# faverogian/diffusion-classifier

Measured on AMD Instinct MI355X. Metric: images classified/sec (node), CIFAR-10 10-class x 50-step ELBO scoring, higher is better.
Workload: dtype bf16; 1 GPU; cifar10-unet-10x50; classes=10, trials=50, forwards_per_image=500, input=uniform [-1,1], parallelism=single

## Files before the change

### diffusion-classifier_amd/csrc/igemm.hip

```cpp
#include <stdio.h>
#include <stdlib.h>
#include "conv3_halo_plan.h"

template <typename T, int BM, int BN, int WGM, int WGN>
__global__ __launch_bounds__(256, 2) void igemm_kernel(const IgemmArgs a) {
  constexpr int EPC = Elem<T>::EPC;
  constexpr int BKE = 8 * EPC;
  constexpr int XL = BM / 32;
  constexpr int WL = (BN + 31) / 32;
  constexpr int WTM = BM / WGM, WTN = BN / WGN;
  constexpr int TM = WTM / 16, TN = WTN / 16;
  static_assert(WGM * WGN == 4, "4 waves");
  extern __shared__ __attribute__((aligned(16))) char smem[];
  constexpr int BUF = (BM + BN) * 128;

  const int t = threadIdx.x;
  const int lane = t & 63, wave = t >> 6;
  const int wm = wave / WGN, wn = wave % WGN;
  const int lr = lane & 15, lq = lane >> 4;

  int tile_m, tile_n;
  tile_of_block(a, tile_m, tile_n);

  const int HWo = a.Hout * a.Wout;
  const int pad = (a.taps == 9) ? 1 : 0;
  const int Hs = a.upsample ? (a.Hin >> 1) : a.Hin;
  const int Ws = a.upsample ? (a.Win >> 1) : a.Win;
  const int chunk = t & 7, lrow = t >> 3;

  int ns0[XL], ns1[XL], iy0[XL], ix0[XL];
#pragma unroll
  for (int i = 0; i < XL; ++i) {
    const int m = tile_m * BM + lrow + 32 * i;
    const bool vm = m < a.M;
    const int mm = vm ? m : 0;
    const int n = mm / HWo;
    const int rem = mm - n * HWo;
    const int oy = rem / a.Wout, ox = rem - oy * a.Wout;
    ns0[i] = a.map0 ? a.map0[n] : n;
    ns1[i] = a.src1 ? (a.map1 ? a.map1[n] : n) : 0;
    iy0[i] = vm ? oy * a.stride - pad : -(1 << 20);
    ix0[i] = ox * a.stride - pad;
  }
  const T* wbase = reinterpret_cast<const T*>(a.W) + (size_t)(tile_n * BN + lrow) * a.Ktot + chunk * EPC;

  chunk16 xr[XL], wr[WL];
  const chunk16 zero = {0u, 0u, 0u, 0u};

  auto load_regs = [&](int ks, int tap, int cc) {
    int ky = 0, kx = 0;
    if (a.taps == 9) { ky = tap / 3; kx = tap - ky * 3; }
    const bool s1 = cc >= a.c0chunks;
    const T* src = reinterpret_cast<const T*>(s1 ? a.src1 : a.src0);
    const int ld = s1 ? a.ld1 : a.ld0;
    const int coff = (s1 ? cc - a.c0chunks : cc) * BKE + chunk * EPC;
#pragma unroll
    for (int i = 0; i < XL; ++i) {
      const int iy = iy0[i] + ky, ix = ix0[i] + kx;
      const bool ok = (unsigned)iy < (unsigned)a.Hin && (unsigned)ix < (unsigned)a.Win;
      const int sy = a.upsample ? (iy >> 1) : iy, sx = a.upsample ? (ix >> 1) : ix;
      const size_t pix = ((size_t)(s1 ? ns1[i] : ns0[i]) * Hs + sy) * Ws + sx;
      xr[i] = zero;
      if (ok) xr[i] = *reinterpret_cast<const chunk16*>(src + pix * ld + coff);
    }
#pragma unroll
    for (int i = 0; i < WL; ++i) {
      if (BN >= 32 * (i + 1) || lrow + 32 * i < BN)
        wr[i] = *reinterpret_cast<const chunk16*>(wbase + (size_t)(32 * i) * a.Ktot + (size_t)ks * BKE);
    }
  };
  auto write_lds = [&](int buf) {
    char* Xs = smem + buf * BUF;
    char* Wsm = Xs + BM * 128;
#pragma unroll
    for (int i = 0; i < XL; ++i) *reinterpret_cast<chunk16*>(Xs + lds_off(lrow + 32 * i, chunk)) = xr[i];
#pragma unroll
    for (int i = 0; i < WL; ++i)
      if (BN >= 32 * (i + 1) || lrow + 32 * i < BN)
        *reinterpret_cast<chunk16*>(Wsm + lds_off(lrow + 32 * i, chunk)) = wr[i];
  };

  f32x4 acc[TN][TM];
#pragma unroll
  for (int i = 0; i < TN; ++i)
#pragma unroll
    for (int j = 0; j < TM; ++j) acc[i][j] = f32x4{0.f, 0.f, 0.f, 0.f};

  int tap = 0, cc = 0;
  load_regs(0, 0, 0);
  write_lds(0);
  __syncthreads();
  for (int ks = 0; ks < a.nk; ++ks) {
    const bool more = ks + 1 < a.nk;
    if (more) {
      if (++cc == a.cpt) { cc = 0; ++tap; }
      load_regs(ks + 1, tap, cc);
    }
    const char* Xs = smem + (ks & 1) * BUF;
    const char* Wsm = Xs + BM * 128;
#pragma unroll
    for (int sub = 0; sub < 2; ++sub) {
      const int c = sub * 4 + lq;
      chunk16 xf[TM], wf[TN];
#pragma unroll
      for (int j = 0; j < TM; ++j) xf[j] = *reinterpret_cast<const chunk16*>(Xs + lds_off(wm * WTM + j * 16 + lr, c));
#pragma unroll
      for (int i = 0; i < TN; ++i) wf[i] = *reinterpret_cast<const chunk16*>(Wsm + lds_off(wn * WTN + i * 16 + lr, c));
#pragma unroll
      for (int i = 0; i < TN; ++i)
#pragma unroll
        for (int j = 0; j < TM; ++j) acc[i][j] = Mma<T>::run(wf[i], xf[j], acc[i][j]);
    }
    if (more) write_lds((ks + 1) & 1);
    __syncthreads();
  }

  igemm_epilogue<TM, TN>(a, acc, tile_m * BM + wm * WTM, tile_n * BN + wn * WTN, lr, lq);
}

template <typename T, int BM, int BN, int WGM, int WGN>
static int launch(const IgemmArgs& a, hipStream_t s) {
  constexpr int lds = 2 * (BM + BN) * 128;
  static bool attr_done = false;
  auto kern = igemm_kernel<T, BM, BN, WGM, WGN>;
  if (!attr_done) {
    (void)hipFuncSetAttribute(reinterpret_cast<const void*>(kern), hipFuncAttributeMaxDynamicSharedMemorySize, lds);
    attr_done = true;
  }
  const long long nblk = (long long)a.tiles_m * a.tiles_n;
  if (nblk <= 0 || nblk > 0x7fffffffLL) { dc_set_error("dc_igemm: bad grid %lld", nblk); return DC_ERR_SHAPE; }
  hipLaunchKernelGGL(kern, dim3((unsigned)nblk), dim3(256), lds, s, a);
  return dc_check_launch("dc_igemm");
}

extern "C" int32_t dc_igemm_cout_pad(int32_t cout, int32_t tile_n) {
  const int tn = tile_n == 32 ? 32 : 128;
  return (cout + tn - 1) / tn * tn;
}


static int igemm_validate_and_fill(const dc_igemm_params* p, IgemmArgs& a) {
  DC_REQUIRE(p, DC_ERR_ARG, "dc_igemm: null params");
  DC_REQUIRE(p->dtype == DC_F32 || p->dtype == DC_BF16 || p->dtype == DC_F16, DC_ERR_DTYPE, "dc_igemm: dtype %d", p->dtype);
  DC_REQUIRE(p->taps == 1 || p->taps == 9, DC_ERR_ARG, "dc_igemm: taps must be 1 or 9 (got %d)", p->taps);
  DC_REQUIRE(p->stride == 1 || p->stride == 2, DC_ERR_ARG, "dc_igemm: stride %d", p->stride);
  DC_REQUIRE(p->tile_n == 128 || p->tile_n == 32, DC_ERR_ARG, "dc_igemm: tile_n %d", p->tile_n);
  DC_REQUIRE(p->src0 && p->W && (p->out || p->pn_out), DC_ERR_ARG, "dc_igemm: null src0/W/out");
  const int bke = 128 / dc_dtype_size(p->dtype);
  DC_REQUIRE(p->C0 > 0 && p->C0 % bke == 0, DC_ERR_SHAPE, "dc_igemm: C0=%d not a multiple of %d", p->C0, bke);
  DC_REQUIRE(p->C1 >= 0 && p->C1 % bke == 0 && ((p->C1 > 0) == (p->src1 != nullptr)), DC_ERR_SHAPE,
             "dc_igemm: C1=%d / src1 mismatch or not a multiple of %d", p->C1, bke);
  DC_REQUIRE(p->n_img > 0 && p->Hout > 0 && p->Wout > 0 && p->Hin > 0 && p->Win > 0 && p->Cout > 0, DC_ERR_SHAPE,
             "dc_igemm: non-positive extent");
  if (p->taps == 9) {
    DC_REQUIRE(p->Hout == (p->Hin + 2 - 3) / p->stride + 1 && p->Wout == (p->Win + 2 - 3) / p->stride + 1, DC_ERR_SHAPE,
               "dc_igemm: 3x3 output %dx%d does not match input %dx%d stride %d", p->Hout, p->Wout, p->Hin, p->Win, p->stride);
  } else {
    DC_REQUIRE(p->stride == 1 && !p->upsample && p->Hout == p->Hin && p->Wout == p->Win, DC_ERR_SHAPE,
               "dc_igemm: taps=1 needs stride 1, no upsample, equal in/out extents");
  }
  if (p->upsample) DC_REQUIRE((p->Hin % 2 == 0) && (p->Win % 2 == 0), DC_ERR_SHAPE, "dc_igemm: upsample needs even Hin/Win");
  const long long M = (long long)p->n_img * p->Hout * p->Wout;
  DC_REQUIRE(M < (1LL << 31), DC_ERR_SHAPE, "dc_igemm: M=%lld too large", M);
  DC_REQUIRE(p->act >= 0 && p->act <= 3, DC_ERR_ARG, "dc_igemm: act %d", p->act);
  if (p->act == DC_ACT_GEGLU) DC_REQUIRE(p->Cout % 32 == 0 && p->tile_n == 128, DC_ERR_SHAPE, "dc_igemm: GEGLU needs Cout%%32==0, tile_n 128");
  if (p->act == DC_ACT_GEGLU) DC_REQUIRE(!p->rowvec, DC_ERR_ARG, "dc_igemm: rowvec cannot be combined with DC_ACT_GEGLU");
  if (p->act == DC_ACT_GEGLU) DC_REQUIRE(!p->gate, DC_ERR_ARG, "dc_igemm: gate cannot be combined with DC_ACT_GEGLU");
  DC_REQUIRE(((uintptr_t)p->src0 & 15) == 0 && ((uintptr_t)p->W & 15) == 0 && ((uintptr_t)p->src1 & 15) == 0, DC_ERR_ALIGN,
             "dc_igemm: src/W must be 16-byte aligned");
  const int epc = 16 / dc_dtype_size(p->dtype);
  DC_REQUIRE(p->ld0 % epc == 0 && p->ld1 % epc == 0 && (p->ld0 == 0 || p->ld0 >= p->C0) && (p->ld1 == 0 || p->ld1 >= p->C1),
             DC_ERR_SHAPE, "dc_igemm: ld0=%d ld1=%d", p->ld0, p->ld1);
  const int cout_out = p->act == DC_ACT_GEGLU ? p->Cout / 2 : p->Cout;
  DC_REQUIRE(p->out_ld >= cout_out, DC_ERR_SHAPE, "dc_igemm: out_ld %d < %d", p->out_ld, cout_out);
  if (p->residual) DC_REQUIRE(p->res_ld >= cout_out, DC_ERR_SHAPE, "dc_igemm: res_ld");
  if (p->rowvec) DC_REQUIRE(p->rowvec_ld >= cout_out, DC_ERR_SHAPE, "dc_igemm: rowvec_ld");
  if (p->gate) DC_REQUIRE(p->gate_ld >= cout_out, DC_ERR_SHAPE, "dc_igemm: gate_ld");

  a.src0 = p->src0; a.map0 = p->map0; a.src1 = p->src1; a.map1 = p->map1; a.W = p->W; a.bias = p->bias;
  a.rowvec = p->rowvec; a.rowvec_map = p->rowvec_map; a.gate = p->gate; a.gate_map = p->gate_map;
  a.residual = p->residual; a.res_map = p->res_map; a.out = p->out;
  a.gn_scale = p->gn_scale; a.gn_shift = p->gn_shift; a.gn_silu = p->gn_silu;
  a.src2 = p->src2; a.map2 = p->map2; a.W2 = p->W2; a.C2 = p->C2; a.ld2 = p->ld2 ? p->ld2 : p->C2;
  a.ln_eps = p->ln_eps; a.qstats = p->qstats;
  a.pn_out = p->pn_out; a.pn_gamma = p->pn_gamma; a.pn_beta = p->pn_beta; a.pn_cnt = reinterpret_cast<unsigned*>(p->pn_cnt);
  a.pn_ld = p->pn_ld ? p->pn_ld : p->Cout; a.pn_groups = p->pn_groups; a.pn_silu = p->pn_silu; a.pn_eps = p->pn_eps;
  DC_REQUIRE((p->gn_scale == nullptr) == (p->gn_shift == nullptr), DC_ERR_ARG, "dc_igemm: gn_scale/gn_shift must both be set or null");
  a.C0 = p->C0; a.C1 = p->C1; a.ld0 = p->ld0 ? p->ld0 : p->C0; a.ld1 = p->ld1 ? p->ld1 : p->C1;
  a.rowvec_ld = p->rowvec_ld; a.gate_ld = p->gate_ld; a.res_dtype = p->res_dtype;
  a.res_ld = p->res_ld; a.out_dtype = p->out_dtype; a.out_ld = p->out_ld; a.act = p->act;
  a.taps = p->taps; a.stride = p->stride; a.upsample = p->upsample; a.Hin = p->Hin; a.Win = p->Win;
  a.Hout = p->Hout; a.Wout = p->Wout; a.Cout = p->Cout;
  a.M = (int)M; a.Ktot = p->taps * (p->C0 + p->C1);
  a.c0chunks = p->C0 / bke; a.cpt = (p->C0 + p->C1) / bke; a.nk = p->taps * a.cpt;
  const int bn = p->tile_n;
  a.tiles_m = (a.M + 127) / 128;
  a.tiles_n = dc_igemm_cout_pad(p->Cout, bn) / bn;
  {
    constexpr long long gemm_cap = 16LL << 20;
    const long long wbytes = (long long)dc_igemm_cout_pad(p->Cout, bn) * a.Ktot * dc_dtype_size(p->dtype);
    a.n_fast = (a.tiles_n > 1 && (wbytes <= (2 << 20) || (p->taps == 1 && wbytes <= gemm_cap))) ? 1 : 0;
  }
  return DC_OK;
}

enum IgemmKernel { IG_THIN, IG_WS, IG_HALO, IG_UP4_HALO, IG_UP4_PIPE, IG_XREG, IG_PIPE, IG_REG128, IG_REG32 };

struct IgemmChoice {
  IgemmKernel kernel = IG_REG32;
  int shape = 0;
  bool gn = false, pn = false;
  int status = DC_OK;
  const char* tag = nullptr;
  const char* message = nullptr;
  HaloPlan halo;
};

static IgemmChoice refuse(const char* tag, const char* message) { return IgemmChoice{IG_REG32, 0, false, false, DC_ERR_UNSUPPORTED, tag, message}; }

static IgemmChoice igemm_choose(const dc_igemm_params* p, const IgemmArgs& a) {
  const int dt = p->dtype, bn = p->tile_n, epc = 16 / dc_dtype_size(dt);
  const int cout_out = p->act == DC_ACT_GEGLU ? p->Cout / 2 : p->Cout;
  const bool lane_epi_ok = cout_out % 8 == 0 && p->out_ld % 8 == 0 && ((uintptr_t)p->out & 15) == 0 &&
                           (!p->residual || (p->res_ld % 8 == 0 && ((uintptr_t)p->residual & 15) == 0)) &&
                           (!p->bias || ((uintptr_t)p->bias & 15) == 0) &&
                           (!p->rowvec || (((uintptr_t)p->rowvec & 15) == 0 && p->rowvec_ld % 4 == 0)) &&
                           (!p->gate || (((uintptr_t)p->gate & 15) == 0 && p->gate_ld % 4 == 0 && p->act == DC_ACT_NONE)) &&
                           (!p->residual || p->res_dtype == dt) && (p->out_dtype == dt || p->out_dtype == DC_F32);
  const bool lds_dma = bn == 128 && lane_epi_ok;
  static const bool no_halo = getenv("DCAMD_NO_HALO") != nullptr;
  const bool halo_ok = lds_dma && !no_halo && dc_conv3_halo_applicable(a, dt);
  const bool qs_args_ok = p->out_dtype == dt && p->Cout % 8 == 0 && ((uintptr_t)a.qstats & 15) == 0;
  const bool pn_args_ok = a.pn_gamma && a.pn_beta && a.pn_cnt && p->out_dtype == dt && a.pn_ld % 8 == 0 && a.pn_ld >= p->Cout &&
                          (((uintptr_t)a.pn_out | (uintptr_t)a.qstats) & 15) == 0 && ((uintptr_t)a.pn_cnt & 3) == 0 && a.pn_eps > 0.f;
  const bool use_pn = a.pn_out != nullptr;

  if (p->up4) {
    const bool up4_halo = lds_dma && !no_halo && !a.src1 && dc_conv3_up4_applicable(a, dt) &&
                          (!a.qstats || (qs_args_ok && (a.Hin >> 1) >= 8 && (a.Win >> 1) >= 8));
    const bool up4_pipe = !up4_halo && lds_dma && !a.src1 && !a.qstats && p->taps == 9 && p->stride == 1 &&
                          p->upsample && p->act == DC_ACT_NONE && !p->gate && !p->residual && !a.gn_scale && !a.src2 &&
                          p->Hin >= 4 && p->Win >= 4 && p->Hin % 2 == 0 && p->Win % 2 == 0 && (p->Hin < 16 || p->Win < 16);
    const HaloPlan plan = up4_halo ? dc_conv3_halo_plan(dc_conv3_up4_walked(a), dt, p->n_img, true) : HaloPlan{};
    if (use_pn && !(up4_halo && a.Hin > 16 && a.Win > 16 && dc_conv3_halo_pn_ok(a, plan, true) && a.qstats && pn_args_ok))
      return refuse("producer-groupnorm-unsupported", "dc_igemm: pn_out given but this upsample conv cannot normalise its own output (see dc_igemm_pn_ok)");
    if (!up4_halo && !up4_pipe)
      return refuse("up4-unsupported", "dc_igemm: up4 given but this problem cannot take the four-phase upsample conv (see dc_igemm_up4_ok)");
    if (up4_halo) return IgemmChoice{IG_UP4_HALO, 0, false, use_pn, DC_OK, nullptr, nullptr, plan};
    return IgemmChoice{IG_UP4_PIPE};
  }

  const bool thin_app = dc_conv3_thin_applicable(a, dt);
  const bool thin = thin_app && ((uintptr_t)p->out & 3) == 0;
  static const bool ws_plain = getenv("DCAMD_WS_PLAIN") != nullptr;
  const bool ws_ok = halo_ok && dc_conv3_ws_ok(a, dt) && !thin_app;
  const bool use_ws = ws_ok && (a.gn_scale || ws_plain);
  const HaloPlan plan = halo_ok && !thin && !use_ws ? dc_conv3_halo_plan(a, dt, p->n_img, false) : HaloPlan{};
  const int bke64 = 64 / dc_dtype_size(dt);
  if (a.src2 && !(halo_ok && (!a.gn_scale || ws_ok) && !a.upsample && a.W2 && a.C2 >= 2 * bke64 && a.C2 % bke64 == 0 && a.ld2 % epc == 0 &&
                  (((uintptr_t)a.src2 | (uintptr_t)a.W2) & 15) == 0))
    return refuse("side-source-unsupported", "dc_igemm: src2/W2 given but this problem cannot take the 1x1 side source (see dc_igemm_side_ok)");
  if (a.gn_scale && !thin && !ws_ok)
    return refuse("gn-not-fusable", "dc_igemm: gn_scale/gn_shift given but this problem cannot take the fused GroupNorm prologue (see dc_igemm_gn_fusable)");
  if (a.qstats && !(halo_ok && !thin_app && qs_args_ok && a.Hin >= 8 && a.Win >= 8))
    return refuse("qstats-unsupported", "dc_igemm: qstats given but this problem cannot emit quad statistics (see dc_igemm_qstats_parts)");
  if (use_pn && !(halo_ok && !use_ws && !a.gn_scale && !thin_app && dc_conv3_halo_pn_ok(a, plan, false) &&
                  (a.qstats || (a.Hin == 4 && a.Win == 4)) && pn_args_ok))
    return refuse("producer-groupnorm-unsupported", "dc_igemm: pn_out given but this problem cannot normalise its own output (see dc_igemm_pn_ok)");
  const bool xreg_app = dc_igemm_xreg_applicable(a, dt);
  if (a.ln_eps > 0.f && !(lds_dma && !a.src1 && xreg_app))
    return refuse("row-layernorm-unsupported", "dc_igemm: ln_eps given but this problem cannot take the fused row LayerNorm (see dc_igemm_ln_ok)");

  if (thin) return IgemmChoice{IG_THIN};
  if (use_ws) return IgemmChoice{IG_WS, 0, a.gn_scale != nullptr};
  if (halo_ok) return IgemmChoice{IG_HALO, 0, false, use_pn, DC_OK, nullptr, nullptr, plan};
  if (!lds_dma) return IgemmChoice{bn == 128 ? IG_REG128 : IG_REG32};
  const int shape = dc_igemm_pipe_shape(a);
  if (xreg_app && (p->act == DC_ACT_GEGLU || a.ln_eps > 0.f || shape != 2)) return IgemmChoice{IG_XREG};
  return IgemmChoice{IG_PIPE, shape};
}

static const char* igemm_name(const IgemmChoice& c, int dtype) {
  static const char* const pipe_fmt[3] = {"igemm_pipe<%s,128x128,2st>", "igemm_pipe<%s,256x128,3st>", "igemm_wide8<%s,256x256>"};
  static thread_local char name[64];
  const char* dn = dtype == DC_BF16 ? "bf16" : (dtype == DC_F16 ? "f16" : "f32");
  switch (c.kernel) {
    case IG_THIN: snprintf(name, sizeof(name), "conv3_thin<%s>", dn); break;
    case IG_WS: snprintf(name, sizeof(name), c.gn ? "conv3_ws<%s,gn>" : "conv3_ws<%s>", dn); break;
    case IG_HALO: snprintf(name, sizeof(name), c.pn ? "conv3_halo<%s,%dw,pn>" : "conv3_halo<%s,%dw>", dn, c.halo.key.NW); break;
    case IG_UP4_HALO: snprintf(name, sizeof(name), c.pn ? "conv3_up4<%s,%dw,pn>" : "conv3_up4<%s,%dw>", dn, c.halo.key.NW); break;
    case IG_UP4_PIPE: snprintf(name, sizeof(name), "igemm_pipe_up4<%s,256x128,3st>", dn); break;
    case IG_XREG: snprintf(name, sizeof(name), "igemm_xreg<%s,96xN>", dn); break;
    case IG_PIPE: snprintf(name, sizeof(name), pipe_fmt[c.shape], dn); break;
    case IG_REG128: snprintf(name, sizeof(name), "igemm<%s,128x128>", dn); break;
    case IG_REG32: snprintf(name, sizeof(name), "igemm<%s,128x32>", dn); break;
  }
  return name;
}

static int igemm_launch(const IgemmChoice& c, const IgemmArgs& a, const dc_igemm_params* p, dc_stream stream) {
  hipStream_t s = reinterpret_cast<hipStream_t>(stream);
  switch (c.kernel) {
    case IG_THIN: return dc_conv3_thin_launch(a, p->dtype, p->n_img, s);
    case IG_WS: return dc_conv3_ws_launch(a, p->dtype, p->n_img, s);
    case IG_HALO: return dc_conv3_halo_launch(c.halo, a, p->dtype, false, s);
    case IG_UP4_HALO: return dc_conv3_halo_launch(c.halo, a, p->dtype, true, s);
    case IG_UP4_PIPE: return dc_igemm_launch_pipe_up4(a, p->dtype, s);
    case IG_XREG: return dc_igemm_xreg_launch(a, p->dtype, s);
    case IG_PIPE: return dc_igemm_launch_pipe(a, p->dtype, c.shape, s);
    case IG_REG128: return dc_by_dtype(p->dtype, "dc_igemm: dtype", [&](auto t) { return launch<decltype(t), 128, 128, 2, 2>(a, s); });
    case IG_REG32: return dc_by_dtype(p->dtype, "dc_igemm: dtype", [&](auto t) { return launch<decltype(t), 128, 32, 4, 1>(a, s); });
  }
  return DC_ERR_ARG;
}

extern "C" int dc_igemm(const dc_igemm_params* p, dc_stream stream) {
  IgemmArgs a;
  const int rc = igemm_validate_and_fill(p, a);
  if (rc != DC_OK) return rc;
  const IgemmChoice c = igemm_choose(p, a);
  if (c.status != DC_OK) { dc_set_error("%s", c.message); return c.status; }
  return igemm_launch(c, a, p, stream);
}

extern "C" const char* dc_igemm_variant(const dc_igemm_params* p) {
  IgemmArgs a;
  if (igemm_validate_and_fill(p, a) != DC_OK) return "invalid";
  const IgemmChoice c = igemm_choose(p, a);
  return c.status == DC_OK ? igemm_name(c, p->dtype) : c.tag;
}

extern "C" const char* dc_igemm_instance(const dc_igemm_params* p, int32_t* geom) {
  IgemmArgs a;
  if (igemm_validate_and_fill(p, a) != DC_OK) return "invalid";
  const IgemmChoice c = igemm_choose(p, a);
  if (c.status != DC_OK) return c.tag;
  static thread_local char name[64];
  const char* dn = p->dtype == DC_BF16 ? "bf16" : (p->dtype == DC_F16 ? "f16" : "f32");
  HaloPlan pl;
  switch (c.kernel) {
    case IG_HALO: case IG_UP4_HALO: {
      pl = c.halo;
      const HaloKey& k = pl.key;
      snprintf(name, sizeof(name), "conv3_halo_kernel<%s,%d,%d,%d%s%s>", dn, k.NW, k.NTAP, k.MODE, k.STG ? ",stag" : "", k.PN ? ",pn" : "");
      break;
    }
    case IG_THIN: pl = dc_conv3_thin_plan(a, p->n_img); snprintf(name, sizeof(name), "conv3_thin_kernel<%s,%s>", dn, a.gn_scale ? "gn" : "plain"); break;
    case IG_WS: pl = dc_conv3_ws_plan(a, p->n_img); snprintf(name, sizeof(name), "conv3_ws_kernel<%s,%s>", dn, a.gn_scale ? "gn" : "plain"); break;
    default: return igemm_name(c, p->dtype);
  }
  if (geom) halo_plan_ints(pl, geom);
  return name;
}

static int32_t igemm_accepts(const dc_igemm_params& q) {
  IgemmArgs a;
  return igemm_validate_and_fill(&q, a) == DC_OK && igemm_choose(&q, a).status == DC_OK ? 1 : 0;
}
alignas(16) static float g_probe_dummy[4] = {0.f, 0.f, 0.f, 0.f};

extern "C" int32_t dc_igemm_gn_fusable(const dc_igemm_params* p) {
  if (!p) return 0;
  dc_igemm_params q = *p;
  q.gn_scale = g_probe_dummy; q.gn_shift = g_probe_dummy;
  return igemm_accepts(q);
}

extern "C" int32_t dc_igemm_ln_ok(const dc_igemm_params* p) {
  if (!p) return 0;
  dc_igemm_params q = *p;
  if (!(q.ln_eps > 0.f)) q.ln_eps = 1e-5f;
  return igemm_accepts(q);
}

extern "C" int32_t dc_igemm_qstats_parts(const dc_igemm_params* p) {
  if (!p) return 0;
  dc_igemm_params q = *p;
  if (!q.qstats) q.qstats = g_probe_dummy;
  if (!igemm_accepts(q)) return 0;
  const int hw = p->Hout * p->Wout;
  if (p->up4) { const int lo = hw >> 2; return 4 * (lo >= 128 ? lo / 128 : 1); }
  return hw >= 128 ? hw / 128 : 1;
}

extern "C" int32_t dc_igemm_pn_ok(const dc_igemm_params* p) {
  if (!p || p->pn_groups <= 0) return 0;
  dc_igemm_params q = *p;
  if (!q.pn_out) q.pn_out = g_probe_dummy;
  if (!q.qstats && !(q.Hin == 4 && q.Win == 4)) q.qstats = g_probe_dummy;
  if (!q.pn_gamma) q.pn_gamma = g_probe_dummy;
  if (!q.pn_beta) q.pn_beta = g_probe_dummy;
  if (!q.pn_cnt) q.pn_cnt = reinterpret_cast<uint32_t*>(g_probe_dummy);
  if (!(q.pn_eps > 0.f)) q.pn_eps = 1e-5f;
  return igemm_accepts(q);
}

extern "C" int32_t dc_pn_timeouts(void) { return (int32_t)dc_conv3_halo_pn_timeouts(); }

struct TailChoice { IgemmArgs a; IgemmChoice c; int status = DC_OK; const char* tag = nullptr; const char* message = nullptr; };

static TailChoice tail_choose(const dc_igemm_params* conv, const dc_pn_tail_params* tail, bool probe) {
  TailChoice t;
  auto fail = [&](int st, const char* tag, const char* msg) -> TailChoice& { t.status = st; t.tag = tag; t.message = msg; return t; };
  if (!conv || !tail) return fail(DC_ERR_ARG, "invalid", "dc_conv3_pn_tail: null params");
  if (conv->out || conv->pn_out) return fail(DC_ERR_UNSUPPORTED, "tail-raw-output", "dc_conv3_pn_tail: the conv's own output (out / pn_out) is never stored; leave both null");
  dc_igemm_params q = *conv;
  q.pn_out = g_probe_dummy;
  q.pn_gamma = tail->gamma; q.pn_beta = tail->beta; q.pn_cnt = tail->cnt;
  q.pn_ld = 0; q.pn_groups = tail->groups; q.pn_silu = tail->silu; q.pn_eps = tail->eps;
  if (probe) {
    if (!q.qstats) q.qstats = g_probe_dummy;
    if (!q.pn_gamma) q.pn_gamma = g_probe_dummy;
    if (!q.pn_beta) q.pn_beta = g_probe_dummy;
    if (!q.pn_cnt) q.pn_cnt = reinterpret_cast<uint32_t*>(g_probe_dummy);
    if (!(q.pn_eps > 0.f)) q.pn_eps = 1e-5f;
  } else if (!tail->Wt || !tail->pred || !tail->ring || ((uintptr_t)tail->Wt & 15) || (((uintptr_t)tail->pred | (uintptr_t)tail->ring | (uintptr_t)tail->bias) & 3)) {
    return fail(DC_ERR_ARG, "invalid", "dc_conv3_pn_tail: Wt (16-byte aligned), pred and ring must be given");
  }
  if (q.pn_groups <= 0) return fail(DC_ERR_ARG, "invalid", "dc_conv3_pn_tail: groups");
  if (igemm_validate_and_fill(&q, t.a) != DC_OK) return fail(DC_ERR_ARG, "invalid", nullptr);
  t.c = igemm_choose(&q, t.a);
  if (t.c.status != DC_OK) return fail(t.c.status, t.c.tag, t.c.message);
  if (t.c.kernel != IG_HALO || !t.c.pn || !dc_conv3_halo_tail_ok(t.a, t.c.halo, q.dtype, tail->Co) || tail->pred_ld < tail->Co)
    return fail(DC_ERR_UNSUPPORTED, "tail-unsupported",
                "dc_conv3_pn_tail: needs a 16-bit 3x3 conv with Cout = 128 on the 4-wave producer-GroupNorm form and 1 <= Co <= 3 (see dc_conv3_pn_tail_ok)");
  return t;
}

extern "C" int32_t dc_conv3_pn_tail_ok(const dc_igemm_params* conv, const dc_pn_tail_params* tail) {
  return tail_choose(conv, tail, true).status == DC_OK ? 1 : 0;
}

extern "C" const char* dc_conv3_pn_tail_variant(const dc_igemm_params* conv, const dc_pn_tail_params* tail) {
  const TailChoice t = tail_choose(conv, tail, true);
  if (t.status != DC_OK) return t.tag;
  return conv->dtype == DC_BF16 ? "conv3_halo<bf16,4w,pn,tail>" : "conv3_halo<f16,4w,pn,tail>";
}

extern "C" int64_t dc_conv3_pn_tail_ring_floats(const dc_igemm_params* conv, const dc_pn_tail_params* tail) {
  const TailChoice t = tail_choose(conv, tail, true);
  if (t.status != DC_OK) return 0;
  const HaloGeom& g = t.c.halo.g;
  return (long long)conv->n_img * g.tiles_x * g.tiles_y * PN_TAIL_RING(1 << g.ltw, 1 << g.lth) * tail->Co;
}

extern "C" int dc_conv3_pn_tail(const dc_igemm_params* conv, const dc_pn_tail_params* tail, dc_stream stream) {
  const TailChoice t = tail_choose(conv, tail, false);
  if (t.status != DC_OK) { if (t.message) dc_set_error("%s", t.message); return t.status; }
  hipStream_t s = reinterpret_cast<hipStream_t>(stream);
  const PnTail tl{tail->Wt, tail->bias, tail->pred, tail->ring, tail->Co, tail->pred_ld};
  const int rc = dc_conv3_halo_tail_launch(t.c.halo, t.a, conv->dtype, tl, s);
  if (rc != DC_OK) return rc;
  const HaloGeom& g = t.c.halo.g;
  return dc_pn_tail_combine_launch(tail->pred, tail->ring, conv->n_img, g.ltw, g.lth, g.tiles_x, g.tiles_y, g.H, g.W, tail->Co, tail->pred_ld, s);
}

extern "C" int32_t dc_igemm_up4_ok(const dc_igemm_params* p) {
  if (!p) return 0;
  dc_igemm_params q = *p;
  q.up4 = 1;
  return igemm_accepts(q);
}

extern "C" int32_t dc_igemm_side_ok(const dc_igemm_params* p) {
  if (!p) return 0;
  dc_igemm_params q = *p;
  if (!q.src2) { q.src2 = g_probe_dummy; q.W2 = g_probe_dummy; }
  return igemm_accepts(q);
}
```

### diffusion-classifier_amd/csrc/igemm_common.h

```cpp
#pragma once
#include "common.h"

struct IgemmArgs {
  const void* src0; const int32_t* map0; const void* src1; const int32_t* map1;
  const void* W; const float* bias;
  const float* rowvec; const int32_t* rowvec_map;
  const float* gate; const int32_t* gate_map;
  const void* residual; const int32_t* res_map;
  void* out;
  const float* gn_scale; const float* gn_shift; int gn_silu;
  const void* src2; const int32_t* map2; const void* W2; int C2, ld2;
  float ln_eps;
  float* qstats;
  void* pn_out; const float* pn_gamma; const float* pn_beta; unsigned* pn_cnt; int pn_ld, pn_groups, pn_silu; float pn_eps;
  int C0, C1, ld0, ld1, rowvec_ld, gate_ld, res_dtype, res_ld, out_dtype, out_ld, act;
  int taps, stride, upsample, Hin, Win, Hout, Wout, Cout;
  int M, Ktot, c0chunks, cpt, nk, tiles_m, tiles_n;
  int n_fast;
};

template <typename T> struct Mma;
template <> struct Mma<__bf16> {
  static __device__ __forceinline__ f32x4 run(const chunk16 w, const chunk16 x, f32x4 acc) {
    return __builtin_amdgcn_mfma_f32_16x16x32_bf16(__builtin_bit_cast(bf16x8, w), __builtin_bit_cast(bf16x8, x), acc, 0, 0, 0);
  }
};
template <> struct Mma<_Float16> {
  static __device__ __forceinline__ f32x4 run(const chunk16 w, const chunk16 x, f32x4 acc) {
    return __builtin_amdgcn_mfma_f32_16x16x32_f16(__builtin_bit_cast(f16x8, w), __builtin_bit_cast(f16x8, x), acc, 0, 0, 0);
  }
};
template <> struct Mma<float> {
  static __device__ __forceinline__ f32x4 run(const chunk16 w, const chunk16 x, f32x4 acc) {
    const f32x4 wf = __builtin_bit_cast(f32x4, w), xf = __builtin_bit_cast(f32x4, x);
    acc = __builtin_amdgcn_mfma_f32_16x16x4f32(wf[0], xf[0], acc, 0, 0, 0);
    acc = __builtin_amdgcn_mfma_f32_16x16x4f32(wf[1], xf[1], acc, 0, 0, 0);
    acc = __builtin_amdgcn_mfma_f32_16x16x4f32(wf[2], xf[2], acc, 0, 0, 0);
    acc = __builtin_amdgcn_mfma_f32_16x16x4f32(wf[3], xf[3], acc, 0, 0, 0);
    return acc;
  }
};

__device__ __forceinline__ int lds_off(int row, int chunk) { return row * 128 + ((chunk ^ ((row >> 1) & 7)) << 4); }

__device__ __forceinline__ void tile_of_block(const IgemmArgs& a, int& tile_m, int& tile_n) {
  const int nblk = gridDim.x, bid = blockIdx.x;
  const int q = nblk >> 3, r = nblk & 7, xcd = bid & 7;
  const int lid = (xcd < r ? xcd * (q + 1) : r * (q + 1) + (xcd - r) * q) + (bid >> 3);
  const bool nf = a.n_fast != 0;
  int tn = a.tiles_n, tm = a.tiles_m;
  asm volatile("" : "+s"(tn), "+s"(tm));
  const int d = nf ? tn : tm;
  const int qt = lid / d, rm = lid - qt * d;
  tile_m = nf ? qt : rm;
  tile_n = nf ? rm : qt;
}

template <int TM, int TN>
__device__ __forceinline__ void igemm_epilogue(const IgemmArgs& a, f32x4 (&acc)[TN][TM], int m0, int n0, int lr, int lq) {
  const int HWo = a.Hout * a.Wout;
  const bool geglu = a.act == DC_ACT_GEGLU;
  const int cout_out = geglu ? (a.Cout >> 1) : a.Cout;
#pragma unroll
  for (int j = 0; j < TM; ++j) {
    const int m = m0 + j * 16 + lr;
    if (m >= a.M) continue;
    const int n = m / HWo;
    const float* rv = a.rowvec ? a.rowvec + (size_t)(a.rowvec_map ? a.rowvec_map[n] : n) * a.rowvec_ld : nullptr;
    const float* gt = a.gate ? a.gate + (size_t)(a.gate_map ? a.gate_map[n] : n) * a.gate_ld : nullptr;
    size_t rrow = 0;
    if (a.residual) rrow = (a.res_map ? (size_t)a.res_map[n] * HWo + (m - n * HWo) : (size_t)m) * a.res_ld;
    const size_t orow = (size_t)m * a.out_ld;
#pragma unroll
    for (int i = 0; i < TN; i += 1) {
      const int pc = n0 + i * 16 + lq * 4;
      float v[4];
      int oc;
      if (geglu) {
        if (i & 1) continue;
        oc = ((n0 + i * 16) >> 1) + lq * 4;
        if (oc >= cout_out) continue;
#pragma unroll
        for (int r = 0; r < 4; ++r) {
          float val = acc[i][j][r], g = acc[(i + 1) % TN][j][r];
          if (a.bias) { val += a.bias[pc + r]; g += a.bias[pc + 16 + r]; }
          v[r] = val * gelu_erf_f(g);
        }
      } else {
        oc = pc;
#pragma unroll
        for (int r = 0; r < 4; ++r) {
          float x = acc[i][j][r];
          const int c = oc + r;
          if (c < cout_out) {
            if (a.bias) x += a.bias[c];
            if (rv) x += rv[c];
            if (a.act == DC_ACT_SILU) x = silu_f(x);
            else if (a.act == DC_ACT_GELU_TANH) x = gelu_tanh_f(x);
            if (gt) x *= gt[c];
          }
          v[r] = x;
        }
      }
      if (oc >= cout_out) continue;
      if (a.residual) {
#pragma unroll
        for (int r = 0; r < 4; ++r)
          if (oc + r < cout_out) v[r] += load_as(a.residual, rrow + oc + r, a.res_dtype);
      }
      if (oc + 3 < cout_out && (a.out_ld & 3) == 0) {
        if (a.out_dtype == DC_F32) {
          *reinterpret_cast<float4*>(reinterpret_cast<float*>(a.out) + orow + oc) = make_float4(v[0], v[1], v[2], v[3]);
        } else if (a.out_dtype == DC_BF16) {
          __bf16 h[4] = {(__bf16)v[0], (__bf16)v[1], (__bf16)v[2], (__bf16)v[3]};
          *reinterpret_cast<uint2*>(reinterpret_cast<__bf16*>(a.out) + orow + oc) = *reinterpret_cast<uint2*>(h);
        } else {
          _Float16 h[4] = {(_Float16)v[0], (_Float16)v[1], (_Float16)v[2], (_Float16)v[3]};
          *reinterpret_cast<uint2*>(reinterpret_cast<_Float16*>(a.out) + orow + oc) = *reinterpret_cast<uint2*>(h);
        }
      } else {
#pragma unroll
        for (int r = 0; r < 4; ++r)
          if (oc + r < cout_out) store_as(a.out, orow + oc + r, a.out_dtype, v[r]);
      }
    }
  }
}

int dc_igemm_pipe_shape(const IgemmArgs& a);
int dc_igemm_launch_pipe(const IgemmArgs& a, int dtype, int shape, hipStream_t s);
int dc_igemm_launch_wide8(const IgemmArgs& a, int dtype, hipStream_t s);
__device__ __forceinline__ void tile_of_block_scalar(const IgemmArgs& a, int& tile_m, int& tile_n) {
  tile_of_block(a, tile_m, tile_n);
  tile_m = __builtin_amdgcn_readfirstlane(tile_m);
  tile_n = __builtin_amdgcn_readfirstlane(tile_n);
  asm volatile("" : "+s"(tile_m), "+s"(tile_n));
}

bool dc_conv3_halo_applicable(const IgemmArgs& a, int dtype);
bool dc_conv3_up4_applicable(const IgemmArgs& a, int dtype);
IgemmArgs dc_conv3_up4_walked(const IgemmArgs& a);
int dc_igemm_launch_pipe_up4(const IgemmArgs& a, int dtype, hipStream_t s);
unsigned dc_conv3_halo_pn_timeouts();
bool dc_conv3_ws_ok(const IgemmArgs& a, int dtype);
int dc_conv3_ws_launch(const IgemmArgs& a, int dtype, int n_img, hipStream_t s);
bool dc_igemm_xreg_applicable(const IgemmArgs& a, int dtype);
int dc_igemm_xreg_launch(const IgemmArgs& a, int dtype, hipStream_t s);
bool dc_conv3_thin_applicable(const IgemmArgs& a, int dtype);
int dc_conv3_thin_launch(const IgemmArgs& a, int dtype, int n_img, hipStream_t s);
```

### diffusion-classifier_amd/csrc/igemm_xreg.hip

```cpp
#include <stdlib.h>
#include "igemm_epilogue.h"
DC_CLOCK_DECL(igemm_xreg)
#ifdef DC_XR_STAMPS
static __device__ unsigned long long* g_xr_stamps;
extern "C" void dc_debug_set_xr_stamps(unsigned long long* p) { (void)hipMemcpyToSymbol(HIP_SYMBOL(g_xr_stamps), &p, sizeof(p)); }
#define XR_NOW() __builtin_amdgcn_s_memtime()
#endif

typedef const __attribute__((address_space(1))) void* gptr_t;
typedef __attribute__((address_space(3))) void* lptr_t;

namespace {
constexpr int XR_TN = 4;
constexpr int XR_R = 4, XR_PD = 3;
constexpr int XR_SLICE = 128 * 128;
constexpr int XR_WL = 4;
}

struct XrPreBias {
  static constexpr bool on = true, has_rowvec = false;
  const float (&v)[8]; const float (&g)[8];
  __device__ __forceinline__ void operator()(int, float (&bs)[8], float (&bgt)[8]) const {
#pragma unroll
    for (int e = 0; e < 8; ++e) { bs[e] = v[e]; bgt[e] = g[e]; }
  }
};

template <int N> static __device__ __forceinline__ void xr_wait_vmcnt() { asm volatile("s_waitcnt vmcnt(%0)" ::"n"(N) : "memory"); }

template <typename T, bool GEGLU, int TM, int KC>
__global__ __launch_bounds__(256, 2) void igemm_xreg_kernel(const IgemmArgs a) {
  static_assert(sizeof(T) == 2, "16-bit operands only");
  constexpr int TN = XR_TN, R = XR_R, PD = XR_PD, WL = XR_WL;
  constexpr int WROWS = TM * 16, XR_BM = 2 * WROWS;
  extern __shared__ __attribute__((aligned(16))) char smem[];
  const int t = threadIdx.x;
  const int lane = t & 63;
  const int wave = __builtin_amdgcn_readfirstlane(t >> 6);
  const int wm = wave >> 1, wn = wave & 1;
  const int lr = lane & 15, lq = lane >> 4;
  const int tile_m = blockIdx.x;
  const int HWo = a.Hout * a.Wout;
  const int kcn = a.Ktot >> 5;
  const int c0c = a.C0 >> 5;
  const int spn = a.Ktot >> 6;
  const int Q = a.tiles_n * spn;

  const int lrow = t >> 3;
  const int lchunk = (t & 7) ^ ((t >> 4) & 7);
  constexpr bool geglu = GEGLU;
  int wro[WL];
#pragma unroll
  for (int i = 0; i < WL; ++i) wro[i] = epi_wrow(lrow + 32 * i, geglu) * a.Ktot + lchunk * 8;
  const T* const Wg = reinterpret_cast<const T*>(a.W);
  int iq = 0, i_nt = 0, i_ks = 0;
  auto issue = [&]() {
    const T* wp = Wg + (size_t)i_nt * 128 * a.Ktot + i_ks * 64;
    char* dst = smem + (iq % R) * XR_SLICE + wave * 1024;
#pragma unroll
    for (int i = 0; i < WL; ++i)
      __builtin_amdgcn_global_load_lds((gptr_t) reinterpret_cast<const char*>(wp + wro[i]), (lptr_t)(dst + i * 4096), 16, 0, 0);
    ++iq;
    if (++i_ks == spn) { i_ks = 0; ++i_nt; }
  };
#pragma unroll
  for (int p = 0; p < PD; ++p)
    if (iq < Q) issue();

  chunk16 xr[TM][KC];
#pragma unroll
  for (int j = 0; j < TM; ++j) {
    const int m = tile_m * XR_BM + wm * WROWS + j * 16 + lr;
    const int mm = m < a.M ? m : a.M - 1;
    const int n = mm / HWo, pix = mm - n * HWo;
    const T* b0 = reinterpret_cast<const T*>(a.src0) + ((size_t)(a.map0 ? a.map0[n] : n) * HWo + pix) * a.ld0 + lq * 8;
    const T* b1 = a.src1 ? reinterpret_cast<const T*>(a.src1) + ((size_t)(a.map1 ? a.map1[n] : n) * HWo + pix) * a.ld1 + lq * 8 : b0;
#pragma unroll
    for (int kc = 0; kc < KC; ++kc) {
      xr[j][kc] = chunk16{0u, 0u, 0u, 0u};
      if (kc < kcn) xr[j][kc] = *reinterpret_cast<const chunk16*>(kc < c0c ? b0 + kc * 32 : b1 + (kc - c0c) * 32);
    }
  }
#pragma unroll
  for (int j = 0; j < TM; ++j)
#pragma unroll
    for (int kc = 0; kc < KC; ++kc) asm volatile("" ::"v"(xr[j][kc]));
  if (a.ln_eps > 0.f) {
    const float invK = 1.0f / (float)a.Ktot;
#pragma unroll
    for (int j = 0; j < TM; ++j) {
      float sum = 0.f;
#pragma unroll
      for (int kc = 0; kc < KC; ++kc)
        if (kc < kcn) {
          float f[8];
          chunk_to_f<T>(xr[j][kc], f);
#pragma unroll
          for (int e = 0; e < 8; ++e) sum += f[e];
        }
      sum += __shfl_xor(sum, 16, 64);
      sum += __shfl_xor(sum, 32, 64);
      const float mean = sum * invK;
      float var = 0.f;
#pragma unroll
      for (int kc = 0; kc < KC; ++kc)
        if (kc < kcn) {
          float f[8];
          chunk_to_f<T>(xr[j][kc], f);
#pragma unroll
          for (int e = 0; e < 8; ++e) var += (f[e] - mean) * (f[e] - mean);
        }
      var += __shfl_xor(var, 16, 64);
      var += __shfl_xor(var, 32, 64);
      const float rstd = rsqrtf(var * invK + a.ln_eps);
#pragma unroll
      for (int kc = 0; kc < KC; ++kc)
        if (kc < kcn) {
          float f[8];
          chunk_to_f<T>(xr[j][kc], f);
#pragma unroll
          for (int e = 0; e < 8; ++e) f[e] = (f[e] - mean) * rstd;
          xr[j][kc] = f_to_chunk<T>(f);
        }
    }
  }
  int landed = iq;

  const uint32_t sbase = lds_addr_of(smem);
  uint32_t woff[2];
#pragma unroll
  for (int sub = 0; sub < 2; ++sub) woff[sub] = sbase + lds_off(wn * 64 + lr, sub * 4 + lq);

  int q = 0;
#ifdef DC_XR_STAMPS
  unsigned long long xs_k = 0, xs_e = 0, xs_t0 = XR_NOW(), xs_w = 0;
#endif
  DC_CLOCK(0);
  for (int nt = 0; nt < a.tiles_n; ++nt) {
    float pbv[8], pbg[8];
#pragma unroll
    for (int e = 0; e < 8; ++e) { pbv[e] = 0.f; pbg[e] = 0.f; }
    if (GEGLU && a.bias) {
      const int c = nt * 64 + wn * 32 + lq * 8;
      if (c < (a.Cout >> 1)) {
        const int p = (c >> 4) * 32 + (c & 15);
        ld8(a.bias + p, pbv);
        ld8(a.bias + p + 16, pbg);
      }
    }
    f32x4 acc[TN][TM];
#pragma unroll
    for (int i = 0; i < TN; ++i)
#pragma unroll
      for (int j = 0; j < TM; ++j) acc[i][j] = f32x4{0.f, 0.f, 0.f, 0.f};
#ifdef DC_XR_STAMPS
    __builtin_amdgcn_sched_barrier(0);
    const unsigned long long xs_a = XR_NOW();
    __builtin_amdgcn_sched_barrier(0);
#endif
#pragma unroll
    for (int ks = 0; ks < KC / 2; ++ks) {
      if (ks < spn) {
#ifdef DC_XR_STAMPS
        __builtin_amdgcn_sched_barrier(0);
        const unsigned long long xs_w0 = XR_NOW();
#endif
        if (q >= landed) {
          const int young = Q - 1 - q;
          if (young >= 2) xr_wait_vmcnt<2 * WL>();
          else if (young == 1) xr_wait_vmcnt<WL>();
          else xr_wait_vmcnt<0>();
        }
        __builtin_amdgcn_s_barrier();
#ifdef DC_XR_STAMPS
        xs_w += XR_NOW() - xs_w0;
        __builtin_amdgcn_sched_barrier(0);
#endif
        if (iq < Q) issue();
        const uint32_t sl = (q % R) * XR_SLICE;
        chunk16 wf[2][TN];
        lgkm_fence0();
#pragma unroll
        for (int sub = 0; sub < 2; ++sub)
#pragma unroll
          for (int i = 0; i < TN; ++i) wf[sub][i] = ds_read16_async(woff[sub] + sl + i * 2048);
#define XR_MMA(SUB, I, NLEFT)                                                                        \
        lgkm_wait<NLEFT>(wf[SUB][I]);                                                                \
        _Pragma("unroll") for (int j = 0; j < TM; ++j) acc[I][j] = Mma<T>::run(wf[SUB][I], xr[j][2 * ks + SUB], acc[I][j]); \
        __builtin_amdgcn_sched_barrier(0);
        XR_MMA(0, 0, 7) XR_MMA(0, 1, 6) XR_MMA(0, 2, 5) XR_MMA(0, 3, 4)
        XR_MMA(1, 0, 3) XR_MMA(1, 1, 2) XR_MMA(1, 2, 1) XR_MMA(1, 3, 0)
#undef XR_MMA
        ++q;
      }
    }
#ifdef DC_XR_STAMPS
    __builtin_amdgcn_sched_barrier(0);
    const unsigned long long xs_b = XR_NOW();
    xs_k += xs_b - xs_a;
    __builtin_amdgcn_sched_barrier(0);
#endif
    auto rowfn = [&](int j, EpiRow& r) {
      const int m = tile_m * XR_BM + wm * WROWS + j * 16 + lr;
      r.ok = m < a.M;
      const int mm = r.ok ? m : a.M - 1;
      const int n = mm / HWo;
      r.samp = n;
      r.o = mm;
      r.r = (a.residual && a.res_map) ? a.res_map[n] * HWo + (mm - n * HWo) : mm;
    };
    const int mw0 = tile_m * XR_BM + wm * WROWS;
    const int sf = min(mw0, a.M - 1) / HWo, sl_ = min(mw0 + WROWS - 1, a.M - 1) / HWo;
    auto drain = [&]() {
      xr_wait_vmcnt<0>();
      landed = iq;
    };
    if constexpr (GEGLU) {
      epi_direct_act<T, TM, DC_ACT_GEGLU, false, true>(a, acc, nt, wn, lq, sf, sl_, rowfn, drain, EpiNoQs(), XrPreBias{pbv, pbg});
    } else {
      epi_direct_act<T, TM, DC_ACT_NONE, false, true>(a, acc, nt, wn, lq, sf, sl_, rowfn, drain);
    }
#ifdef DC_XR_STAMPS
    __builtin_amdgcn_sched_barrier(0);
    xs_e += XR_NOW() - xs_b;
    __builtin_amdgcn_sched_barrier(0);
#endif
  }
#ifdef DC_XR_STAMPS
  if (threadIdx.x == 0 && g_xr_stamps) {
    g_xr_stamps[blockIdx.x * 4] = xs_k; g_xr_stamps[blockIdx.x * 4 + 1] = xs_e; g_xr_stamps[blockIdx.x * 4 + 2] = XR_NOW() - xs_t0; g_xr_stamps[blockIdx.x * 4 + 3] = xs_w;
  }
#endif
  DC_CLOCK(1);
}

bool dc_igemm_xreg_applicable(const IgemmArgs& a, int dtype) {
  static const bool off = getenv("DCAMD_NO_XREG") != nullptr;
  if (off || dtype == DC_F32 || a.taps != 1 || a.gate) return false;
  if (a.act != DC_ACT_NONE && a.act != DC_ACT_GEGLU) return false;
  if (a.rowvec && a.Hout * a.Wout < 48) return false;
  constexpr int min_tiles = 3;
  if (a.tiles_n < min_tiles) return false;
  if (a.Ktot > 512 || (a.Ktot & 63) || (a.C0 & 31) || (a.C1 & 31)) return false;
  return true;
}

template <typename T, int TM, int KC>
static int xreg_launch_t(const IgemmArgs& a0, hipStream_t s) {
  constexpr int lds = XR_R * XR_SLICE;
  IgemmArgs a = a0;
  a.tiles_m = (a.M + 2 * TM * 16 - 1) / (2 * TM * 16);
  static bool attr_done[2] = {false, false};
  const bool gg = a.act == DC_ACT_GEGLU;
  void (*kern)(const IgemmArgs) = gg ? igemm_xreg_kernel<T, true, TM, KC> : igemm_xreg_kernel<T, false, TM, KC>;
  if (!attr_done[gg ? 1 : 0]) {
    (void)hipFuncSetAttribute(reinterpret_cast<const void*>(kern), hipFuncAttributeMaxDynamicSharedMemorySize, lds);
    attr_done[gg ? 1 : 0] = true;
  }
  hipLaunchKernelGGL(kern, dim3((unsigned)a.tiles_m), dim3(256), lds, s, a);
  return dc_check_launch("dc_igemm(xreg)");
}

int dc_igemm_xreg_launch(const IgemmArgs& a, int dtype, hipStream_t s) {
  return dc_by_dtype16(dtype, "dc_igemm: dtype", [&](auto t) {
    return a.Ktot <= 256 ? xreg_launch_t<decltype(t), 3, 8>(a, s) : xreg_launch_t<decltype(t), 2, 16>(a, s);
  });
}
```

Baseline: 231.1 images/s.

## Add K-specialised xreg GEGLU kernel with compile-time slice pipeline and hoisted row indexing

Adds a template variant of the xreg igemm kernel that is specialised on the number of K slices for the GEGLU projection (Ktot 256 or 512). The weight-load ring is fully unrolled with compile-time slots and offsets, vmcnt waits are computed statically, and prefetching runs across N-tile boundaries. Epilogue row indices are also hoisted out of the N-tile loop. The intent is to remove runtime queue bookkeeping, address arithmetic and per-tile index recomputation, at the cost of more kernel instantiations and possibly more register pressure.

```diff
diff --git a/diffusion-classifier_amd/csrc/igemm.hip b/diffusion-classifier_amd/csrc/igemm.hip
--- a/diffusion-classifier_amd/csrc/igemm.hip
+++ b/diffusion-classifier_amd/csrc/igemm.hip
@@ -347,6 +347,10 @@
     }
     case IG_THIN: pl = dc_conv3_thin_plan(a, p->n_img); snprintf(name, sizeof(name), "conv3_thin_kernel<%s,%s>", dn, a.gn_scale ? "gn" : "plain"); break;
     case IG_WS: pl = dc_conv3_ws_plan(a, p->n_img); snprintf(name, sizeof(name), "conv3_ws_kernel<%s,%s>", dn, a.gn_scale ? "gn" : "plain"); break;
+    case IG_XREG:
+      snprintf(name, sizeof(name), "igemm_xreg_kernel<%s,%s,%s,%d>", dn, a.act == DC_ACT_GEGLU ? "geglu" : "plain", a.Ktot <= 256 ? "3,8" : "2,16",
+               dc_igemm_xreg_spn(a));
+      return name;
     default: return igemm_name(c, p->dtype);
   }
   if (geom) halo_plan_ints(pl, geom);
diff --git a/diffusion-classifier_amd/csrc/igemm_common.h b/diffusion-classifier_amd/csrc/igemm_common.h
--- a/diffusion-classifier_amd/csrc/igemm_common.h
+++ b/diffusion-classifier_amd/csrc/igemm_common.h
@@ -146,5 +146,6 @@
 int dc_conv3_ws_launch(const IgemmArgs& a, int dtype, int n_img, hipStream_t s);
 bool dc_igemm_xreg_applicable(const IgemmArgs& a, int dtype);
 int dc_igemm_xreg_launch(const IgemmArgs& a, int dtype, hipStream_t s);
+int dc_igemm_xreg_spn(const IgemmArgs& a);
 bool dc_conv3_thin_applicable(const IgemmArgs& a, int dtype);
 int dc_conv3_thin_launch(const IgemmArgs& a, int dtype, int n_img, hipStream_t s);
diff --git a/diffusion-classifier_amd/csrc/igemm_xreg.hip b/diffusion-classifier_amd/csrc/igemm_xreg.hip
--- a/diffusion-classifier_amd/csrc/igemm_xreg.hip
+++ b/diffusion-classifier_amd/csrc/igemm_xreg.hip
@@ -1,4 +1,5 @@
 #include <stdlib.h>
+#include <utility>
 #include "igemm_epilogue.h"
 DC_CLOCK_DECL(igemm_xreg)
 #ifdef DC_XR_STAMPS
@@ -27,10 +28,24 @@
 };
 
 template <int N> static __device__ __forceinline__ void xr_wait_vmcnt() { asm volatile("s_waitcnt vmcnt(%0)" ::"n"(N) : "memory"); }
-
-template <typename T, bool GEGLU, int TM, int KC>
+template <int... I, typename F> static __device__ __forceinline__ void xr_unrolled(std::integer_sequence<int, I...>, F&& f) { (f(EpiIC<I>{}), ...); }
+
+template <int SLOT, int OFF, bool IN_LOOP>
+static __device__ __forceinline__ void xr_issue_at(const char* base, uint32_t (&wrb)[XR_WL], char* ring_wave) {
+  const char* sb = base + OFF;
+  asm volatile("" : "+s"(sb));
+#pragma unroll
+  for (int i = 0; i < XR_WL; ++i) {
+    if constexpr (IN_LOOP) asm volatile("" : "+v"(wrb[i]));
+    __builtin_amdgcn_global_load_lds((gptr_t)(sb + wrb[i]), (lptr_t)(ring_wave + SLOT * XR_SLICE + i * 4096), 16, 0, 0);
+  }
+}
+
+template <typename T, bool GEGLU, int TM, int KC, int SPN = 0>
 __global__ __launch_bounds__(256, 2) void igemm_xreg_kernel(const IgemmArgs a) {
   static_assert(sizeof(T) == 2, "16-bit operands only");
+  static_assert(SPN == 0 || (2 * SPN == KC && SPN % XR_R == 0 && SPN > XR_PD), "K-specialised form: whole rings of slices per N tile");
+  constexpr int KT = SPN * 64;
   constexpr int TN = XR_TN, R = XR_R, PD = XR_PD, WL = XR_WL;
   constexpr int WROWS = TM * 16, XR_BM = 2 * WROWS;
   extern __shared__ __attribute__((aligned(16))) char smem[];
@@ -41,8 +56,12 @@
   const int lr = lane & 15, lq = lane >> 4;
   const int tile_m = blockIdx.x;
   const int HWo = a.Hout * a.Wout;
-  const int kcn = a.Ktot >> 5;
-  const int c0c = a.C0 >> 5;
+  int kcn = a.Ktot >> 5;
+  int c0c = a.C0 >> 5;
+  if constexpr (SPN != 0) {
+    asm volatile("" : "+s"(kcn));
+    asm volatile("" : "+s"(c0c));
+  }
   const int spn = a.Ktot >> 6;
   const int Q = a.tiles_n * spn;
 
@@ -53,6 +72,13 @@
 #pragma unroll
   for (int i = 0; i < WL; ++i) wro[i] = epi_wrow(lrow + 32 * i, geglu) * a.Ktot + lchunk * 8;
   const T* const Wg = reinterpret_cast<const T*>(a.W);
+  uint32_t wrb[WL] = {};
+  if constexpr (SPN != 0) {
+#pragma unroll
+    for (int i = 0; i < WL; ++i) wrb[i] = (uint32_t)(epi_wrow(lrow + 32 * i, geglu) * KT + lchunk * 8) * 2u;
+  }
+  const char* const Wb = reinterpret_cast<const char*>(a.W);
+  char* const ring_wave = smem + wave * 1024;
   int iq = 0, i_nt = 0, i_ks = 0;
   auto issue = [&]() {
     const T* wp = Wg + (size_t)i_nt * 128 * a.Ktot + i_ks * 64;
@@ -63,9 +89,17 @@
     ++iq;
     if (++i_ks == spn) { i_ks = 0; ++i_nt; }
   };
-#pragma unroll
-  for (int p = 0; p < PD; ++p)
-    if (iq < Q) issue();
+  if constexpr (SPN != 0) {
+    xr_unrolled(std::make_integer_sequence<int, PD>{}, [&](auto pc) {
+      constexpr int p = decltype(pc)::value;
+      xr_issue_at<p % R, p * 128, false>(Wb, wrb, ring_wave);
+    });
+    iq = PD;
+  } else {
+#pragma unroll
+    for (int p = 0; p < PD; ++p)
+      if (iq < Q) issue();
+  }
 
   chunk16 xr[TM][KC];
 #pragma unroll
@@ -135,6 +169,28 @@
 #ifdef DC_XR_STAMPS
   unsigned long long xs_k = 0, xs_e = 0, xs_t0 = XR_NOW(), xs_w = 0;
 #endif
+  auto rowfn = [&](int j, EpiRow& r) {
+    const int m = tile_m * XR_BM + wm * WROWS + j * 16 + lr;
+    r.ok = m < a.M;
+    const int mm = r.ok ? m : a.M - 1;
+    const int n = mm / HWo;
+    r.samp = n;
+    r.o = mm;
+    r.r = (a.residual && a.res_map) ? a.res_map[n] * HWo + (mm - n * HWo) : mm;
+  };
+  int h_o[TM] = {}, h_r[TM] = {}, h_n[TM] = {};
+  int h_sf = 0, h_sl = 0;
+  if constexpr (SPN != 0) {
+#pragma unroll
+    for (int j = 0; j < TM; ++j) {
+      EpiRow r;
+      rowfn(j, r);
+      h_o[j] = r.ok ? r.o : -1; h_r[j] = r.r; h_n[j] = r.samp;
+    }
+    const int mw0 = tile_m * XR_BM + wm * WROWS;
+    h_sf = min(mw0, a.M - 1) / HWo; h_sl = min(mw0 + WROWS - 1, a.M - 1) / HWo;
+  }
+  auto rowfn_h = [&](int j, EpiRow& r) { r.ok = h_o[j] >= 0; r.o = h_o[j]; r.r = h_r[j]; r.samp = h_n[j]; };
   DC_CLOCK(0);
   for (int nt = 0; nt < a.tiles_n; ++nt) {
     float pbv[8], pbg[8];
@@ -158,67 +214,95 @@
     const unsigned long long xs_a = XR_NOW();
     __builtin_amdgcn_sched_barrier(0);
 #endif
-#pragma unroll
-    for (int ks = 0; ks < KC / 2; ++ks) {
-      if (ks < spn) {
-#ifdef DC_XR_STAMPS
-        __builtin_amdgcn_sched_barrier(0);
-        const unsigned long long xs_w0 = XR_NOW();
-#endif
-        if (q >= landed) {
-          const int young = Q - 1 - q;
-          if (young >= 2) xr_wait_vmcnt<2 * WL>();
-          else if (young == 1) xr_wait_vmcnt<WL>();
-          else xr_wait_vmcnt<0>();
-        }
-        __builtin_amdgcn_s_barrier();
-#ifdef DC_XR_STAMPS
-        xs_w += XR_NOW() - xs_w0;
-        __builtin_amdgcn_sched_barrier(0);
-#endif
-        if (iq < Q) issue();
-        const uint32_t sl = (q % R) * XR_SLICE;
-        chunk16 wf[2][TN];
-        lgkm_fence0();
-#pragma unroll
-        for (int sub = 0; sub < 2; ++sub)
-#pragma unroll
-          for (int i = 0; i < TN; ++i) wf[sub][i] = ds_read16_async(woff[sub] + sl + i * 2048);
 #define XR_MMA(SUB, I, NLEFT)                                                                        \
         lgkm_wait<NLEFT>(wf[SUB][I]);                                                                \
         _Pragma("unroll") for (int j = 0; j < TM; ++j) acc[I][j] = Mma<T>::run(wf[SUB][I], xr[j][2 * ks + SUB], acc[I][j]); \
         __builtin_amdgcn_sched_barrier(0);
-        XR_MMA(0, 0, 7) XR_MMA(0, 1, 6) XR_MMA(0, 2, 5) XR_MMA(0, 3, 4)
+#define XR_SLICE_MMAS(READ)                                                                          \
+        chunk16 wf[2][TN];                                                                           \
+        lgkm_fence0();                                                                               \
+        READ                                                                                         \
+        XR_MMA(0, 0, 7) XR_MMA(0, 1, 6) XR_MMA(0, 2, 5) XR_MMA(0, 3, 4)                              \
         XR_MMA(1, 0, 3) XR_MMA(1, 1, 2) XR_MMA(1, 2, 1) XR_MMA(1, 3, 0)
+    if constexpr (SPN != 0) {
+      const bool last = nt == a.tiles_n - 1;
+      const char* const wt = Wb + (size_t)nt * (128 * KT * 2);
+      xr_unrolled(std::make_integer_sequence<int, SPN>{}, [&](auto ksc) {
+        constexpr int ks = decltype(ksc)::value;
+#ifdef DC_XR_STAMPS
+        __builtin_amdgcn_sched_barrier(0);
+        const unsigned long long xs_w0 = XR_NOW();
+#endif
+        if constexpr (ks >= PD) {
+          constexpr int young_last = SPN - 1 - ks;
+          if constexpr (young_last >= PD - 1) xr_wait_vmcnt<(PD - 1) * WL>();
+          else if (last) xr_wait_vmcnt<young_last * WL>();
+          else xr_wait_vmcnt<(PD - 1) * WL>();
+        }
+        __builtin_amdgcn_s_barrier();
+#ifdef DC_XR_STAMPS
+        xs_w += XR_NOW() - xs_w0;
+        __builtin_amdgcn_sched_barrier(0);
+#endif
+        constexpr int is = ks + PD;
+        if constexpr (is < SPN) xr_issue_at<is % R, is * 128, true>(wt, wrb, ring_wave);
+        else if (!last) xr_issue_at<is % R, 128 * KT * 2 + (is - SPN) * 128, true>(wt, wrb, ring_wave);
+        constexpr int sl = (ks % R) * XR_SLICE;
+        XR_SLICE_MMAS(xr_unrolled(std::make_integer_sequence<int, 2 * TN>{}, [&](auto rc) {
+          constexpr int sub = decltype(rc)::value / TN, i = decltype(rc)::value % TN;
+          wf[sub][i] = ds_read16_async_off<sl + i * 2048>(woff[sub]);
+        });)
+      });
+    } else {
+#pragma unroll
+      for (int ks = 0; ks < KC / 2; ++ks) {
+        if (ks < spn) {
+#ifdef DC_XR_STAMPS
+          __builtin_amdgcn_sched_barrier(0);
+          const unsigned long long xs_w0 = XR_NOW();
+#endif
+          if (q >= landed) {
+            const int young = Q - 1 - q;
+            if (young >= 2) xr_wait_vmcnt<2 * WL>();
+            else if (young == 1) xr_wait_vmcnt<WL>();
+            else xr_wait_vmcnt<0>();
+          }
+          __builtin_amdgcn_s_barrier();
+#ifdef DC_XR_STAMPS
+          xs_w += XR_NOW() - xs_w0;
+          __builtin_amdgcn_sched_barrier(0);
+#endif
+          if (iq < Q) issue();
+          const uint32_t sl = (q % R) * XR_SLICE;
+          XR_SLICE_MMAS(_Pragma("unroll") for (int sub = 0; sub < 2; ++sub)
+                          _Pragma("unroll") for (int i = 0; i < TN; ++i) wf[sub][i] = ds_read16_async(woff[sub] + sl + i * 2048);)
+          ++q;
+        }
+      }
+    }
+#undef XR_SLICE_MMAS
 #undef XR_MMA
-        ++q;
-      }
-    }
 #ifdef DC_XR_STAMPS
     __builtin_amdgcn_sched_barrier(0);
     const unsigned long long xs_b = XR_NOW();
     xs_k += xs_b - xs_a;
     __builtin_amdgcn_sched_barrier(0);
 #endif
-    auto rowfn = [&](int j, EpiRow& r) {
-      const int m = tile_m * XR_BM + wm * WROWS + j * 16 + lr;
-      r.ok = m < a.M;
-      const int mm = r.ok ? m : a.M - 1;
-      const int n = mm / HWo;
-      r.samp = n;
-      r.o = mm;
-      r.r = (a.residual && a.res_map) ? a.res_map[n] * HWo + (mm - n * HWo) : mm;
-    };
-    const int mw0 = tile_m * XR_BM + wm * WROWS;
-    const int sf = min(mw0, a.M - 1) / HWo, sl_ = min(mw0 + WROWS - 1, a.M - 1) / HWo;
     auto drain = [&]() {
       xr_wait_vmcnt<0>();
       landed = iq;
     };
-    if constexpr (GEGLU) {
-      epi_direct_act<T, TM, DC_ACT_GEGLU, false, true>(a, acc, nt, wn, lq, sf, sl_, rowfn, drain, EpiNoQs(), XrPreBias{pbv, pbg});
+    if constexpr (SPN != 0) {
+      static_assert(SPN == 0 || GEGLU, "the K-specialised form is instantiated for the GEGLU projection only");
+      epi_direct_act<T, TM, DC_ACT_GEGLU, false, true>(a, acc, nt, wn, lq, h_sf, h_sl, rowfn_h, drain, EpiNoQs(), XrPreBias{pbv, pbg});
     } else {
-      epi_direct_act<T, TM, DC_ACT_NONE, false, true>(a, acc, nt, wn, lq, sf, sl_, rowfn, drain);
+      const int mw0 = tile_m * XR_BM + wm * WROWS;
+      const int sf = min(mw0, a.M - 1) / HWo, sl_ = min(mw0 + WROWS - 1, a.M - 1) / HWo;
+      if constexpr (GEGLU) {
+        epi_direct_act<T, TM, DC_ACT_GEGLU, false, true>(a, acc, nt, wn, lq, sf, sl_, rowfn, drain, EpiNoQs(), XrPreBias{pbv, pbg});
+      } else {
+        epi_direct_act<T, TM, DC_ACT_NONE, false, true>(a, acc, nt, wn, lq, sf, sl_, rowfn, drain);
+      }
     }
 #ifdef DC_XR_STAMPS
     __builtin_amdgcn_sched_barrier(0);
@@ -245,17 +329,25 @@
   return true;
 }
 
+int dc_igemm_xreg_spn(const IgemmArgs& a) {
+  if (a.act != DC_ACT_GEGLU || (a.Ktot != 256 && a.Ktot != 512) || getenv("DCAMD_XREG_NO_KSPEC") != nullptr) return 0;
+  return a.Ktot >> 6;
+}
+
 template <typename T, int TM, int KC>
 static int xreg_launch_t(const IgemmArgs& a0, hipStream_t s) {
   constexpr int lds = XR_R * XR_SLICE;
   IgemmArgs a = a0;
   a.tiles_m = (a.M + 2 * TM * 16 - 1) / (2 * TM * 16);
-  static bool attr_done[2] = {false, false};
+  static bool attr_done[3] = {false, false, false};
   const bool gg = a.act == DC_ACT_GEGLU;
-  void (*kern)(const IgemmArgs) = gg ? igemm_xreg_kernel<T, true, TM, KC> : igemm_xreg_kernel<T, false, TM, KC>;
-  if (!attr_done[gg ? 1 : 0]) {
+  const bool kspec = dc_igemm_xreg_spn(a) == KC / 2;
+  const int which = kspec ? 2 : gg ? 1 : 0;
+  void (*kern)(const IgemmArgs) = kspec ? igemm_xreg_kernel<T, true, TM, KC, KC / 2>
+                                  : gg  ? igemm_xreg_kernel<T, true, TM, KC> : igemm_xreg_kernel<T, false, TM, KC>;
+  if (!attr_done[which]) {
     (void)hipFuncSetAttribute(reinterpret_cast<const void*>(kern), hipFuncAttributeMaxDynamicSharedMemorySize, lds);
-    attr_done[gg ? 1 : 0] = true;
+    attr_done[which] = true;
   }
   hipLaunchKernelGGL(kern, dim3((unsigned)a.tiles_m), dim3(256), lds, s, a);
   return dc_check_launch("dc_igemm(xreg)");
```

Result: no change. 233.2 images/s, median of 6 (+0.9%).
